# noah-aviel-dove/signals

Measured on AMD Instinct MI355X. Metric: rendered Msamples/s (48 kHz, 256-sample blocks), higher is better.
Workload: dtype f64; 1 GPU; C2: 1024-voice Fixed->Sine->LowPass->Gain->SumBus(stereo) per GPU, 48 kHz, 256-frame blocks, 4096 blocks per batch (f32 storage, f64 phase/recurrence); engine schedule = fused voice chain + bus: sig_fused_voice_bus (Sine->LowPass->Gain->SumBus in ONE launch, its voice tiles added in fixed order by the same kernel; no per-voice sample touches HBM); voices_per_gpu=1024, block_frames=256, start_position=0, parallelism=voices sharded 1024/GPU x1; single process, no collective, rccl_ranks=0

## Files before the change

signals_amd/csrc/fused_voice.hip:

```cpp
#include <cstdlib>

#include "sig_fused_launch.h"

sig_fused::Tuning& sig_fused::tuning() {
    static Tuning t = [] {
        auto env = [](const char* name, int dflt) { const char* e = getenv(name); return e ? atoi(e) : dflt; };
        Tuning u;
        u.vpt = env("SIG_FUSED_VPT", 0); u.span = env("SIG_FUSED_SPAN", 0);
        u.steady = env("SIG_FUSED_STEADY", -1); u.scan = env("SIG_FUSED_SCAN", -1);
        if (u.steady == 2) { u.steady = 1; u.tile_sum_kernel = 1; }
        if (u.steady == 3) { u.steady = 1; u.mix_f32 = 1; }
        return u;
    }();
    return t;
}

namespace {

enum Sink { SINK_VOICES, SINK_MIX, SINK_BUS };
struct FusedCall {
    int osc_kind, filt_type; int32_t rate; int64_t position;
    int32_t block_frames, nblocks, context, voices;
    const double* hertz; int32_t hertz_stride; const double* phase; int32_t phase_stride;
    const double* cutoff; int32_t cutoff_stride; const double* gain; int32_t gain_stride;
    float* out; int64_t out_ld; int32_t* status; void* stream;
    Sink sink = SINK_VOICES;
    bool rows = false;
    int32_t cutoff_rows = 1, gain_rows = 1;
    int pair_op = 0, kind2 = 0;
    const double* hertz2 = nullptr; int32_t hertz2_stride = 0; const double* phase2 = nullptr; int32_t phase2_stride = 0;
    const double* mix = nullptr; int32_t mix_stride = 0;
    int32_t hertz_rows = 1, phase_rows = 1; const double* hertz_hist = nullptr; const double* phase_hist = nullptr;
    bool devpos = false; const int64_t* position_dev = nullptr;
    const float* matrix = nullptr;
    const double* bus_gains = nullptr; int64_t bus_gains_ld = 0; int32_t bus_channels = 0; double* workspace = nullptr;
    double* consts = nullptr; int32_t consts_ready = 0; int force_walk = 0;
};

bool stride_ok(int32_t s) { return (s | 1) == 1; }

bool call_ok(const FusedCall& c)
{
    const bool bus = c.sink == SINK_BUS;
    if (c.filt_type != SIG_FILT_LOWPASS && c.filt_type != SIG_FILT_HIGHPASS) return false;
    if (!(c.rate > 0 && (c.devpos ? c.position_dev != nullptr : c.position >= 0))) return false;
    if (!(c.block_frames >= 0 && c.nblocks >= 0 && c.context >= 0 && c.voices >= 0)) return false;
    if (!(c.hertz && c.cutoff && c.out && c.out_ld >= (bus ? c.bus_channels : c.voices))) return false;
    if (!(stride_ok(c.hertz_stride) && stride_ok(c.phase_stride) && stride_ok(c.cutoff_stride) && stride_ok(c.gain_stride))) return false;
    if (!((c.cutoff_rows == 1 || c.cutoff_rows == c.nblocks) && (c.gain_rows == 1 || c.gain_rows == c.nblocks))) return false;
    if (c.pair_op != 0 && !((c.pair_op == 1 || c.pair_op == 2) && c.kind2 >= SIG_OSC_SINE && c.kind2 <= SIG_OSC_TRIANGLE && c.hertz2 &&
                            stride_ok(c.hertz2_stride) && stride_ok(c.phase2_stride) && stride_ok(c.mix_stride) && (c.pair_op == 2 || c.mix)))
        return false;
    if ((c.hertz_hist || c.phase_hist) && c.block_frames < c.context) return false;
    if (!((c.hertz_rows == 1 || (c.hertz_rows == c.nblocks && c.hertz_hist)) &&
          (c.phase_rows == 1 || (c.phase_rows == c.nblocks && c.phase_hist)) && (!c.phase_hist || c.phase))) return false;
    if (c.sink == SINK_MIX && !(c.matrix && c.voices % 64 == 0)) return false;
    if (bus && !(c.workspace && (c.bus_gains ? c.bus_gains_ld >= c.voices : c.bus_channels == 1))) return false;
    return true;
}

int run_call(const FusedCall& c)
{
    SIG_CHECK_ARG(call_ok(c));
    if (c.block_frames == 0 || c.nblocks == 0 || c.voices == 0) return 0;
    const bool bus = c.sink == SINK_BUS;
    FusedArgs a{c.filt_type, (double)c.rate, c.devpos ? 0 : c.position, c.block_frames, c.nblocks, c.context, c.voices,
                c.hertz, c.hertz_stride, c.phase, c.phase_stride, c.cutoff, c.cutoff_stride, c.gain, c.gain_stride,
                bus ? nullptr : c.out, bus ? 0 : c.out_ld, 0, c.status, c.devpos ? c.position_dev : nullptr};
    a.mix = c.matrix;
    a.consts_ext = c.consts; a.consts_ready = c.consts_ready; a.force_walk = c.force_walk;
    a.cutoff_rows = c.cutoff_rows; a.gain_rows = c.gain_rows;
    a.hertz_rows = c.hertz_rows; a.phase_rows = c.phase_rows; a.hertz_hist = c.hertz_hist; a.phase_hist = c.phase_hist;
    a.pair_op = c.pair_op; a.kind2 = c.kind2; a.hertz2 = c.hertz2; a.hs2 = c.hertz2_stride; a.phase2 = c.phase2; a.ps2 = c.phase2_stride;
    a.mixrow = c.mix; a.ms = c.mix_stride;
    const BusArgs busargs = bus ? BusArgs{c.bus_gains, c.bus_gains_ld, c.workspace, (int64_t)c.block_frames * c.nblocks}
                                : BusArgs{nullptr, 0, nullptr, 0};
    hipStream_t s = static_cast<hipStream_t>(c.stream);
    if (c.rows) {
        SIG_CHECK_ARG(!bus || c.bus_channels == 1 || c.bus_channels == 2);
        return dispatch_rows(bus ? c.bus_channels : 0, c.osc_kind, a, busargs, c.out, c.out_ld, s);
    }
    switch (c.sink) {
        case SINK_BUS: return dispatch_bus(c.gain != nullptr, c.osc_kind, c.bus_channels, a, busargs, c.out, c.out_ld, s);
        case SINK_MIX: return dispatch_mix(c.gain != nullptr, c.osc_kind, a, s);
        default: return dispatch_chain(c.gain != nullptr, c.osc_kind, a, s);
    }
}

void set_rows(FusedCall& c, int32_t cutoff_rows, int32_t gain_rows) { c.rows = true; c.cutoff_rows = cutoff_rows; c.gain_rows = gain_rows; }

void set_bus(FusedCall& c, const double* bus_gains, int64_t bus_gains_ld, int32_t bus_channels, double* workspace)
{
    c.sink = SINK_BUS; c.bus_gains = bus_gains; c.bus_gains_ld = bus_gains_ld; c.bus_channels = bus_channels; c.workspace = workspace;
}
// ... 107 lines not shown
                                      int32_t block_frames, int32_t nblocks, int32_t context, int32_t voices,
                                      const double* hertz, int32_t hertz_stride, int32_t hertz_rows, const double* hertz_hist,
                                      const double* phase, int32_t phase_stride, int32_t phase_rows, const double* phase_hist,
                                      const double* cutoff, int32_t cutoff_stride, int32_t cutoff_rows,
                                      const double* gain, int32_t gain_stride, int32_t gain_rows,
                                      const double* bus_gains, int64_t bus_gains_ld, int32_t bus_channels,
                                      double* workspace, float* out, int64_t out_ld, int32_t* status, void* stream)
{
    FusedCall c{osc_kind, filt_type, rate, position, block_frames, nblocks, context, voices, hertz, hertz_stride, phase, phase_stride,
                cutoff, cutoff_stride, gain, gain_stride, out, out_ld, status, stream};
    set_rows(c, cutoff_rows, gain_rows);
    set_fm(c, hertz_rows, hertz_hist, phase_rows, phase_hist);
    set_bus(c, bus_gains, bus_gains_ld, bus_channels, workspace);
    return run_call(c);
}

extern "C" int sig_fused_osc_biquad_devpos(int osc_kind, int filt_type, int32_t rate, const int64_t* position_dev,
                                           int32_t block_frames, int32_t nblocks, int32_t context, int32_t voices,
                                           const double* hertz, int32_t hertz_stride, const double* phase, int32_t phase_stride,
                                           const double* cutoff, int32_t cutoff_stride,
                                           const double* gain, int32_t gain_stride,
                                           float* out, int64_t out_ld, int32_t* status, void* stream)
{
    FusedCall c{osc_kind, filt_type, rate, 0, block_frames, nblocks, context, voices, hertz, hertz_stride, phase, phase_stride,
                cutoff, cutoff_stride, gain, gain_stride, out, out_ld, status, stream};
    c.devpos = true; c.position_dev = position_dev;
    return run_call(c);
}

namespace {
__global__ void advance_kernel(int64_t* p, int64_t delta) { *p += delta; }
}

extern "C" int sig_advance_position(int64_t* position_dev, int64_t delta, void* stream)
{
    SIG_CHECK_ARG(position_dev != nullptr);
    advance_kernel<<<1, 1, 0, static_cast<hipStream_t>(stream)>>>(position_dev, delta);
    return sig_launch_status();
}

extern "C" int sig_fused_osc_biquad_mix(int osc_kind, int filt_type, int32_t rate, int64_t position,
                                        int32_t block_frames, int32_t nblocks, int32_t context, int32_t voices,
                                        const double* hertz, int32_t hertz_stride, const double* phase, int32_t phase_stride,
                                        const double* cutoff, int32_t cutoff_stride,
                                        const double* gain, int32_t gain_stride,
                                        const float* matrix, float* out, int64_t out_ld, int32_t* status, void* stream)
{
    FusedCall c{osc_kind, filt_type, rate, position, block_frames, nblocks, context, voices, hertz, hertz_stride, phase, phase_stride,
                cutoff, cutoff_stride, gain, gain_stride, out, out_ld, status, stream};
    c.sink = SINK_MIX; c.matrix = matrix;
    return run_call(c);
}

extern "C" int sig_fused_geometry(int32_t voices, int32_t block_frames, int32_t nblocks, int32_t context,
                                  int32_t* voices_per_lane, int32_t* blocks_per_lane)
{
    SIG_CHECK_ARG(voices >= 0 && block_frames >= 0 && nblocks >= 0 && context >= 0 && voices_per_lane && blocks_per_lane);
    FusedArgs a{};
    a.N = block_frames; a.K = nblocks; a.ctx = context; a.voices = voices;
    int vpt = 1, span = 1;
    pick_geometry(a, 4, vpt, span);
    *voices_per_lane = vpt;
    *blocks_per_lane = span;
    return 0;
}

extern "C" int sig_fused_voice_bus_plan(int osc_kind, int64_t position, int32_t voices, int32_t block_frames, int32_t nblocks,
                                       int32_t context, int32_t* voices_per_lane, int32_t* blocks_per_lane,
                                       int32_t* closed_form)
{
    SIG_CHECK_ARG(voices >= 0 && block_frames >= 0 && nblocks >= 0 && context >= 0 && position >= 0);
    SIG_CHECK_ARG(voices_per_lane && blocks_per_lane && closed_form);
    FusedArgs a{};
    a.position = position; a.N = block_frames; a.K = nblocks; a.ctx = context; a.voices = voices;
    const BusPlan p = plan_voice_bus(a, osc_kind);
    *voices_per_lane = p.vpt;
    *blocks_per_lane = p.span;
    *closed_form = p.steady;
    return 0;
}

extern "C" int sig_fused_set_tuning(int32_t voices_per_lane, int32_t blocks_per_lane, int32_t closed_form, int32_t scan)
{
    SIG_CHECK_ARG(voices_per_lane >= 0 && blocks_per_lane >= 0 && closed_form >= -1 && closed_form <= 3 && scan >= -1);
    Tuning& t = tuning();
    t.vpt = voices_per_lane; t.span = blocks_per_lane; t.scan = scan;
    t.steady = (closed_form == 2 || closed_form == 3) ? 1 : closed_form;
    t.tile_sum_kernel = (closed_form == 2) ? 1 : 0;
    t.mix_f32 = (closed_form == 3) ? 1 : 0;
    return 0;
}

extern "C" int64_t sig_fused_voice_bus_workspace(int32_t voices, int64_t rows, int32_t bus_channels)
{
    return (steady_consts_offset(voices, rows, bus_channels) + (int64_t)kSteadyConsts * voices) * (int64_t)sizeof(double);
}

extern "C" int sig_fused_voice_bus(int osc_kind, int filt_type, int32_t rate, int64_t position,
                                   int32_t block_frames, int32_t nblocks, int32_t context, int32_t voices,
                                   const double* hertz, int32_t hertz_stride, const double* phase, int32_t phase_stride,
                                   const double* cutoff, int32_t cutoff_stride,
                                   const double* gain, int32_t gain_stride,
                                   const double* bus_gains, int64_t bus_gains_ld, int32_t bus_channels,
                                   double* workspace, float* out, int64_t out_ld, int32_t* status, void* stream)
{
    FusedCall c{osc_kind, filt_type, rate, position, block_frames, nblocks, context, voices, hertz, hertz_stride, phase, phase_stride,
                cutoff, cutoff_stride, gain, gain_stride, out, out_ld, status, stream};
    set_bus(c, bus_gains, bus_gains_ld, bus_channels, workspace);
    return run_call(c);
}

extern "C" int sig_fused_voice_bus_walk(int osc_kind, int filt_type, int32_t rate, int64_t position,
                                        int32_t block_frames, int32_t nblocks, int32_t context, int32_t voices,
                                        const double* hertz, int32_t hertz_stride, const double* phase, int32_t phase_stride,
                                        const double* cutoff, int32_t cutoff_stride,
                                        const double* gain, int32_t gain_stride,
                                        const double* bus_gains, int64_t bus_gains_ld, int32_t bus_channels,
                                        double* workspace, float* out, int64_t out_ld, int32_t* status, void* stream)
{
    FusedCall c{osc_kind, filt_type, rate, position, block_frames, nblocks, context, voices, hertz, hertz_stride, phase, phase_stride,
                cutoff, cutoff_stride, gain, gain_stride, out, out_ld, status, stream};
    set_bus(c, bus_gains, bus_gains_ld, bus_channels, workspace);
    c.force_walk = 1;
    return run_call(c);
}

extern "C" int64_t sig_fused_voice_consts_size(int32_t voices)
{
    return (int64_t)kSteadyConsts * voices * (int64_t)sizeof(double);
}

extern "C" int sig_fused_voice_bus_prepared(int osc_kind, int filt_type, int32_t rate, int64_t position,
                                            int32_t block_frames, int32_t nblocks, int32_t context, int32_t voices,
                                            const double* hertz, int32_t hertz_stride, const double* phase, int32_t phase_stride,
                                            const double* cutoff, int32_t cutoff_stride,
                                            const double* gain, int32_t gain_stride,
                                            const double* bus_gains, int64_t bus_gains_ld, int32_t bus_channels,
                                            double* workspace, float* out, int64_t out_ld, int32_t* status, void* stream,
                                            double* consts, int32_t consts_ready)
{
    SIG_CHECK_ARG(consts != nullptr);
    FusedCall c{osc_kind, filt_type, rate, position, block_frames, nblocks, context, voices, hertz, hertz_stride, phase, phase_stride,
                cutoff, cutoff_stride, gain, gain_stride, out, out_ld, status, stream};
    set_bus(c, bus_gains, bus_gains_ld, bus_channels, workspace);
    c.consts = consts; c.consts_ready = consts_ready;
    return run_call(c);
}

extern "C" int sig_fused_voice_bus_bound(const sig_fused_voice_bus_call* b, int64_t position, float* out, int32_t consts_ready,
                                         int32_t walk, void* stream)
{
    SIG_CHECK_ARG(b != nullptr && (walk || b->consts != nullptr));
    FusedCall c{b->osc_kind, b->filt_type, b->rate, position, b->block_frames, b->nblocks, b->context, b->voices, b->hertz, b->hertz_stride,
                b->phase, b->phase_stride, b->cutoff, b->cutoff_stride, b->gain, b->gain_stride, out, b->out_ld, b->status, stream};
    set_bus(c, b->bus_gains, b->bus_gains_ld, b->bus_channels, b->workspace);
    if (walk) c.force_walk = 1;
    else { c.consts = b->consts; c.consts_ready = consts_ready; }
    return run_call(c);
}
```

signals_amd/csrc/sig_fused_steady.h:

```cpp
#pragma once
#include <type_traits>

#include "sig_biquad.h"
#include "sig_bus_tile.h"
#include "sig_osc.h"
#include "sig_steady.h"

namespace {

using namespace sig_fused;
using sig_bus::kPairs;
using sig_bus::kTileStride;

enum { SC_NA1, SC_NA2, SC_SCALE, SC_K2C, SC_ST, SC_CT, SC_HRE, SC_HIM, SC_ND, SC_T, SC_T0 = SC_T + 4, kSteadyConsts = SC_T0 + 4 };

__device__ __forceinline__ bool steady_wave(const FusedArgs& a, int v0, int vpt, int64_t p0, int nb) {
    const double q_first = (double)p0 / a.rate, q_last = (double)(p0 + (int64_t)nb * a.N - 1) / a.rate;
    bool ok = true;
    for (int i = 0; i < vpt; ++i) {
        const int v = (v0 + i < a.voices) ? v0 + i : ((v0 < a.voices) ? v0 : 0);
        ok &= steady_voice_ok(a.hertz[(int64_t)v * a.hs], a.phase ? a.phase[(int64_t)v * a.ps] : 0.0, a.rate,
                              a.steady_consts[(int64_t)SC_ST * a.voices + v], q_first, q_last);
    }
    return __all(ok);
}

template <bool GAIN>
__global__ __launch_bounds__(256) void steady_prep_kernel(FusedArgs a, double* __restrict__ consts)
{
    const int v = blockIdx.x * blockDim.x + threadIdx.x;
    if (v >= a.voices) return;
    const SteadyVoice c = steady_constants<GAIN>(a, v);
    if (!c.ok && a.status) atomicOr(a.status, SIG_STATUS_BAD_CUTOFF);
    auto put = [&](int k, double x) { consts[(int64_t)k * a.voices + v] = x; };
    put(SC_NA1, c.na1); put(SC_NA2, c.na2); put(SC_SCALE, c.scale);
    put(SC_K2C, c.k2c); put(SC_ST, c.st); put(SC_CT, c.ct);
    put(SC_HRE, c.hre); put(SC_HIM, c.him); put(SC_ND, c.nd);
    put(SC_T + 0, c.T.a); put(SC_T + 1, c.T.b); put(SC_T + 2, c.T.c); put(SC_T + 3, c.T.d);
    put(SC_T0 + 0, c.T0.a); put(SC_T0 + 1, c.T0.b); put(SC_T0 + 2, c.T0.c); put(SC_T0 + 3, c.T0.d);
}

template <int VPT, int C>
__device__ __forceinline__ void steady_fallback_span(const FusedArgs& a, const BusArgs& bus, double* tile, int lane, int vt,
                                                  int64_t b_first, int nb, int v0)
{
    const int vc = (v0 < a.voices) ? v0 : 0;
    const double* sc = a.steady_consts;
    const double s2 = (a.type == SIG_FILT_LOWPASS) ? 2.0 : -2.0;
    sig_bus::PipelinedTile<C> stage(tile, lane, bus.partials + (int64_t)vt * bus.rows * C, b_first * a.N);
    for (int i = 0; i < VPT; ++i)
        if (v0 + i < a.voices && a.status && sc[(int64_t)SC_NA1 * a.voices + v0 + i] != sc[(int64_t)SC_NA1 * a.voices + v0 + i])
            atomicOr(a.status, SIG_STATUS_BAD_CUTOFF);
#pragma unroll 1
    for (int bi = 0; bi < nb; ++bi) {
        const int64_t p_b = a.position + (b_first + bi) * a.N;
        const int c = (int)((p_b < (int64_t)a.ctx) ? p_b : (int64_t)a.ctx);
        double z0[VPT], z1[VPT];
#pragma unroll
        for (int i = 0; i < VPT; ++i) z0[i] = z1[i] = 0.0;
#pragma unroll 1
        for (int r = -c; r < a.N; ++r) {
            const double q = (double)(p_b + r) / a.rate;
            double acc[C];
#pragma unroll
            for (int ch = 0; ch < C; ++ch) acc[ch] = 0.0;
#pragma unroll
            for (int i = 0; i < VPT; ++i) {
                const bool live = v0 + i < a.voices;
                const int v = live ? v0 + i : vc;
                const double t = q * a.hertz[(int64_t)v * a.hs] + (a.phase ? a.phase[(int64_t)v * a.ps] : 0.0);
                const double x = (double)sig_osc::osc_sine_f32(t);
                double na1 = sc[(int64_t)SC_NA1 * a.voices + v], na2 = sc[(int64_t)SC_NA2 * a.voices + v];
                double scale = live ? sc[(int64_t)SC_SCALE * a.voices + v] : 0.0;
                if (a.cutoff_rows > 1) {
                    Biquad qd;
                    design_butter2(a.type, a.cutoff[(b_first + bi) * (int64_t)(a.cs ? a.voices : 1) + (int64_t)v * a.cs], a.rate, qd);
                    na1 = -qd.a1; na2 = -qd.a2;
                    scale = live ? qd.b0 : 0.0;
                    if (a.gain && a.gain_rows == 1) scale *= a.gain[(int64_t)v * a.gs];
                }
                const double y = x + z0[i];
                z0[i] = fma(na1, y, fma(s2, x, z1[i]));
                z1[i] = fma(na2, y, x);
                if (a.gain_rows > 1) scale *= a.gain[(b_first + bi) * (int64_t)(a.gs ? a.voices : 1) + (int64_t)v * a.gs];
#pragma unroll
                for (int ch = 0; ch < C; ++ch) acc[ch] = fma(bus.pan ? bus.pan[ch * bus.pan_ld + v] * scale : scale, y, acc[ch]);
            }
            if (r >= 0) {
#pragma unroll
                for (int ch = 0; ch < C; ++ch) stage.slot[ch * kTileStride] = acc[ch];
                stage.advance();
            }
        }
    }
    if (stage.staged) stage.now();
}

template <int VPT> struct SteadyVariants {
    static constexpr int count = (VPT >= 8) ? 7 : (VPT == 4) ? 4 : (VPT == 2) ? 3 : 2;
    static constexpr int at(int k) {
        constexpr int v8[7] = {8, 6, 4, 3, 2, 1, 0}, v4[4] = {4, 2, 1, 0}, v2[3] = {2, 1, 0}, v1[2] = {1, 0};
        return (VPT >= 8) ? v8[k] : (VPT == 4) ? v4[k] : (VPT == 2) ? v2[k] : v1[k];
    }
};

#ifndef SIG_STEADY_OCC8
#define SIG_STEADY_OCC8 1
#endif
#ifndef SIG_STEADY_AUTO16
#define SIG_STEADY_AUTO16 0
#endif
#ifndef SIG_STEADY_OCC16
#define SIG_STEADY_OCC16 1
#endif
template <int VPT> struct SteadyOcc { static constexpr int waves = (VPT == 16) ? SIG_STEADY_OCC16 : (VPT == 8) ? SIG_STEADY_OCC8 : 2; };

template <int VPT, int C, bool GROWS, bool CROWS = false>
__device__ __forceinline__ void steady_bus_wave(const FusedArgs& a, const BusArgs& bus, double* tile, int lane, int wave, double* osc_store = nullptr)
{
    constexpr bool OSC_LDS = CROWS && VPT >= 8;
    constexpr int R = kPairs / C;
    constexpr int LC = SteadyVariants<VPT>::at(0);
    static_assert(R % 2 == 0, "the two-term recurrence rotates two registers per voice: row groups are even");
    const int64_t item = (int64_t)blockIdx.x * 4 + wave;
    const int vt = (int)(item % a.voice_tiles);
    const int64_t b_first = (item / a.voice_tiles) * a.span;
    if (b_first >= a.K) return;
    const int nb = (int)((a.K - b_first < (int64_t)a.span) ? a.K - b_first : (int64_t)a.span);
    const int v0 = (vt * SIG_WAVE + lane) * VPT;
    const int vc = (v0 < a.voices) ? v0 : 0;
    const int64_t p0 = a.position + b_first * a.N;
    if (!steady_wave(a, v0, VPT, p0, nb)) {
        steady_fallback_span<VPT, C>(a, bus, tile, lane, vt, b_first, nb, v0);
        return;
    }
    const double* sc = a.steady_consts;

    double na1[LC], na2[LC], k2c[VPT], ya[VPT], yb[VPT], wt[C][VPT];
    int nd_total[VPT];
    const double q_first = (double)p0 / a.rate;
#pragma unroll
    for (int i = 0; i < VPT; ++i) {
        const bool live = v0 + i < a.voices;
        const int v = live ? v0 + i : vc;
        auto cst = [&](int k) { return sc[(int64_t)k * a.voices + v]; };
        const double na1_i = cst(SC_NA1);
        if (i < LC) { na1[i < LC ? i : 0] = na1_i; na2[i < LC ? i : 0] = cst(SC_NA2); }
        k2c[i] = cst(SC_K2C);
        if (live && na1_i != na1_i && a.status) atomicOr(a.status, SIG_STATUS_BAD_CUTOFF);
        const double scale = cst(SC_SCALE);
#pragma unroll
        for (int ch = 0; ch < C; ++ch)
            wt[ch][i] = live ? (bus.pan ? bus.pan[ch * bus.pan_ld + v] * scale : scale) : 0.0;
        const double hz = a.hertz[(int64_t)v * a.hs], ph = a.phase ? a.phase[(int64_t)v * a.ps] : 0.0;
        const double t_first = q_first * hz + ph;
        const double f0 = t_first - rint(t_first);
        const double ur = sin2pi(f0 + 0.25), ui = sin2pi(f0);
        const double hre = cst(SC_HRE), him = cst(SC_HIM);
        const double wr = fma(hre, ur, -(him * ui)), wi = fma(hre, ui, him * ur);
        yb[i] = wi;
        ya[i] = fma(wi, cst(SC_CT), -(wr * cst(SC_ST)));
        const double nd = cst(SC_ND);
        nd_total[i] = (live && nd < (double)kNeverDrops) ? (int)nd : (live ? kNeverDrops : 0);
    }
#pragma unroll
    for (int d = 1; d < SIG_WAVE; d <<= 1) {
        int other[VPT];
#pragma unroll
        for (int i = 0; i < VPT; ++i) other[i] = __shfl_xor(nd_total[i], d, SIG_WAVE);
#pragma unroll
        for (int i = 0; i < VPT; ++i) nd_total[i] = (other[i] > nd_total[i]) ? other[i] : nd_total[i];
    }
#pragma unroll
    for (int i = 0; i < VPT; ++i) nd_total[i] = __builtin_amdgcn_readfirstlane(nd_total[i]);

    double* dstp = bus.partials + (int64_t)vt * bus.rows * C;
    sig_bus::PipelinedTile<C> stage(tile, lane, dstp, b_first * a.N);

    if constexpr (LC < VPT) {
        const int c_min = (b_first == 0 && a.position < (int64_t)a.ctx) ? (int)a.position : a.ctx;
        bool capped = true;
#pragma unroll
        for (int i = LC; i < VPT; ++i) capped &= nd_total[i] <= c_min;
        if (!capped) {
            steady_fallback_span<VPT, C>(a, bus, tile, lane, vt, b_first, nb, v0);
            return;
        }
    }
    [[maybe_unused]] OscPart osc[(CROWS && !OSC_LDS) ? VPT : 1];
    auto osc_slot = [&](int field, int i) -> double& { return osc_store[((size_t)field * VPT + i) * SIG_WAVE + lane]; };
    if constexpr (CROWS) {
#pragma unroll
        for (int i = 0; i < VPT; ++i) {
            const int v = (v0 + i < a.voices) ? v0 + i : vc;
            const OscPart made = steady_osc_part(a.type, a.hertz[(int64_t)v * a.hs], a.rate, a.ctx);
            if constexpr (OSC_LDS) {
                osc_slot(0, i) = made.ct; osc_slot(1, i) = made.st; osc_slot(2, i) = made.beta; osc_slot(3, i) = made.enr; osc_slot(4, i) = made.eni;
            } else {
                osc[i] = made;
            }
        }
    }
    double z0h[LC], z1h[LC];
    auto row = [&](double* sums, int sums_stride, auto m_tag, auto odd_tag) {
        constexpr int M = decltype(m_tag)::value;
        constexpr bool ODD = decltype(odd_tag)::value;
        double y[VPT];
#pragma unroll
        for (int i = 0; i < VPT; ++i) {
            const double ys = ODD ? ya[i] : yb[i];
            if (ODD) yb[i] = fma(k2c[i], ya[i], -yb[i]);
            else ya[i] = fma(k2c[i], yb[i], -ya[i]);
            if (i < M) {
                const int j = i < LC ? i : 0;
                y[i] = ys + z0h[j];
                const double yh = z0h[j];
                z0h[j] = fma(na1[j], yh, z1h[j]);
                z1h[j] = na2[j] * yh;
            } else {
                y[i] = ys;
            }
        }
#pragma unroll
        for (int ch = 0; ch < C; ++ch) {
            double acc = 0.0;
#pragma unroll
            for (int i = 0; i < VPT; ++i) acc = fma(wt[ch][i], y[i], acc);
            sums[ch * sums_stride] = acc;
        }
    };
    sig_bus::FoldedGroup<C> folded(tile, lane, dstp);
    double pend[4];
    int64_t pend_row = 0;
    bool have = false;
    auto rows2 = [&](double* sums, auto m_tag) {
        constexpr int M = decltype(m_tag)::value;
        double y0[VPT], y1[VPT];
#pragma unroll
        for (int i = 0; i < VPT; ++i) {
            y0[i] = yb[i];
            ya[i] = fma(k2c[i], yb[i], -ya[i]);
            y1[i] = ya[i];
            yb[i] = fma(k2c[i], ya[i], -yb[i]);
            if (i < M) {
                const int j = i < LC ? i : 0;
                const double h0 = z0h[j];
                y0[i] += h0;
                const double h1 = fma(na1[j], h0, z1h[j]);
                y1[i] += h1;
                z0h[j] = fma(na1[j], h1, na2[j] * h0);
                z1h[j] = na2[j] * h1;
            }
        }
        double acc0[C], acc1[C];
#pragma unroll
        for (int ch = 0; ch < C; ++ch) { acc0[ch] = 0.0; acc1[ch] = 0.0; }
#pragma unroll
        for (int i = 0; i < VPT; ++i) {
#pragma unroll
            for (int ch = 0; ch < C; ++ch) {
                acc0[ch] = fma(wt[ch][i], y0[i], acc0[ch]);
                acc1[ch] = fma(wt[ch][i], y1[i], acc1[ch]);
            }
        }
#pragma unroll
        for (int ch = 0; ch < C; ++ch) { sums[ch] = acc0[ch]; sums[C + ch] = acc1[ch]; }
    };
    auto group = [&](auto m_tag) {
        double acc[kPairs];
#pragma unroll
        for (int k = 0; k < R; k += 2) {
            rows2(acc + k * C, m_tag);
#pragma unroll
            for (int q = 0; q < kPairs / 4; ++q)
                if (4 * q + 3 < (k + 2) * C && 4 * q + 3 >= k * C)
                    folded.fold4(q, acc[4 * q], acc[4 * q + 1], acc[4 * q + 2], acc[4 * q + 3]);
            if (k + 2 == R / 2 && have) folded.finish(pend, pend_row, R);
        }
        folded.issue(pend);
        pend_row = stage.first; stage.first += R; have = true;
    };
    using Variants = SteadyVariants<VPT>;

    for (int bi = 0; bi < nb; ++bi) {
        if constexpr (GROWS && !CROWS) {
#pragma unroll
            for (int i = 0; i < VPT; ++i) {
                const bool live = v0 + i < a.voices;
                const int v = live ? v0 + i : vc;
                const double scale = sc[(int64_t)SC_SCALE * a.voices + v] * a.gain[(b_first + bi) * (int64_t)(a.gs ? a.voices : 1) + (int64_t)v * a.gs];
#pragma unroll
                for (int ch = 0; ch < C; ++ch) wt[ch][i] = live ? (bus.pan ? bus.pan[ch * bus.pan_ld + v] * scale : scale) : 0.0;
            }
        }
        const bool first = (b_first + bi == 0);
        const int tk = first ? SC_T0 : SC_T;
        const int c = first ? (int)((a.position < (int64_t)a.ctx) ? a.position : (int64_t)a.ctx) : a.ctx;
        if constexpr (CROWS) {
            const int64_t blk = b_first + bi;
            const double q_b = (double)(p0 + (int64_t)bi * a.N) / a.rate;
            double cut_i[VPT], gain_i[VPT];
#pragma unroll
            for (int i = 0; i < VPT; ++i) {
                const int v = (v0 + i < a.voices) ? v0 + i : vc;
                cut_i[i] = a.cutoff[(a.cutoff_rows > 1 ? blk * (int64_t)(a.cs ? a.voices : 1) : 0) + (int64_t)v * a.cs];
                gain_i[i] = a.gain ? a.gain[(a.gain_rows > 1 ? blk * (int64_t)(a.gs ? a.voices : 1) : 0) + (int64_t)v * a.gs] : 1.0;
            }
#pragma unroll
            for (int i = 0; i < VPT; ++i) {
                const bool live = v0 + i < a.voices;
                const int v = live ? v0 + i : vc;
                const double cutoff = cut_i[i], gain = gain_i[i];
                const double hz_v = a.hertz[(int64_t)v * a.hs], ph_v = a.phase ? a.phase[(int64_t)v * a.ps] : 0.0;
                OscPart op;
                if constexpr (OSC_LDS) op = OscPart{osc_slot(0, i), osc_slot(1, i), osc_slot(2, i), osc_slot(3, i), osc_slot(4, i)};
                else op = osc[i];
                if (__builtin_expect(c != a.ctx, 0)) op = steady_osc_part(a.type, hz_v, a.rate, c);
                const double ct_i = op.ct, st_i = op.st;
                const BlockVoice cv = steady_block_constants(a.type, a.rate, cutoff, gain, op, c);
                if (i < LC) { na1[i < LC ? i : 0] = cv.na1; na2[i < LC ? i : 0] = cv.na2; }
                if (live && !cv.ok && a.status) atomicOr(a.status, SIG_STATUS_BAD_CUTOFF);
#pragma unroll
                for (int ch = 0; ch < C; ++ch) wt[ch][i] = live ? (bus.pan ? bus.pan[ch * bus.pan_ld + v] * cv.scale : cv.scale) : 0.0;
                const double t_first = q_b * hz_v + ph_v;
                const double f0 = t_first - rint(t_first);
                const double ur = sin2pi(f0 + 0.25), ui = sin2pi(f0);
                const double wr = fma(cv.hre, ur, -(cv.him * ui)), wi = fma(cv.hre, ui, cv.him * ur);
                yb[i] = wi;
                ya[i] = fma(wi, ct_i, -(wr * st_i));
                if (i < LC) {
                    const double dss = fma(k2c[i], yb[i], -ya[i]) - yb[i];
                    z0h[i < LC ? i : 0] = fma(cv.T.a, yb[i], cv.T.b * dss);
                    z1h[i < LC ? i : 0] = fma(cv.T.c, yb[i], cv.T.d * dss);
                }
                nd_total[i] = (live && cv.nd < (double)kNeverDrops) ? (int)cv.nd : (live ? kNeverDrops : 0);
            }
#pragma unroll
            for (int d = 1; d < SIG_WAVE; d <<= 1) {
                int other[VPT];
#pragma unroll
                for (int i = 0; i < VPT; ++i) other[i] = __shfl_xor(nd_total[i], d, SIG_WAVE);
#pragma unroll
                for (int i = 0; i < VPT; ++i) nd_total[i] = (other[i] > nd_total[i]) ? other[i] : nd_total[i];
            }
#pragma unroll
            for (int i = 0; i < VPT; ++i) nd_total[i] = __builtin_amdgcn_readfirstlane(nd_total[i]);
        }
        int drop_at[LC];
#pragma unroll
        for (int i = 0; i < LC; ++i) {
            drop_at[i] = (nd_total[i] > c) ? nd_total[i] - c : 0;
            if (drop_at[i] > 0) {
                const int v = (v0 + i < a.voices) ? v0 + i : vc;
                const double dss = fma(k2c[i], yb[i], -ya[i]) - yb[i];
                if constexpr (!CROWS) {
                    const double* t = sc + (int64_t)tk * a.voices + v;
                    z0h[i] = fma(t[0], yb[i], t[a.voices] * dss);
                    z1h[i] = fma(t[2 * (int64_t)a.voices], yb[i], t[3 * (int64_t)a.voices] * dss);
                }
            } else {
                z0h[i] = 0.0; z1h[i] = 0.0;
            }
        }
        int done = 0;
        auto single = [&]() {
            row(stage.slot, kTileStride, std::integral_constant<int, LC>{}, std::false_type{});
#pragma unroll
            for (int i = 0; i < VPT; ++i) { const double t = ya[i]; ya[i] = yb[i]; yb[i] = t; }
            ++done;
            stage.advance();
        };
        while (stage.staged != 0 && done < a.N) single();
        const int last_group_row = done + ((a.N - done) / R) * R;
        auto phase = [&](auto k_tag) {
            constexpr int K = decltype(k_tag)::value;
            constexpr int M = Variants::at(K);
            constexpr int lower = (K + 1 < Variants::count) ? Variants::at(K + 1) : 0;
            int until = 0;
#pragma unroll
            for (int i = lower; i < LC; ++i) until = (i < M && drop_at[i] > until) ? drop_at[i] : until;
            if (M == 0) until = a.N;
            until = (until < last_group_row) ? until : last_group_row;
            while (done < until) {
                group(std::integral_constant<int, M>{});
                done += R;
            }
        };
#define SIG_PHASE(K) if constexpr (K < Variants::count) phase(std::integral_constant<int, K>{});
        SIG_PHASE(0) SIG_PHASE(1) SIG_PHASE(2) SIG_PHASE(3) SIG_PHASE(4) SIG_PHASE(5) SIG_PHASE(6) SIG_PHASE(7) SIG_PHASE(8)
#undef SIG_PHASE
        if (done < a.N) {
            if (have) { folded.finish(pend, pend_row, R); have = false; }
#pragma unroll
            for (int i = 0; i < LC; ++i)
                if (drop_at[i] <= done) { z0h[i] = 0.0; z1h[i] = 0.0; }
            while (done < a.N) single();
        }
    }
    if (have) folded.finish(pend, pend_row, R);
    if (stage.staged) stage.now();
}

template <int VPT, int C, bool GROWS = false, bool CROWS = false>
__global__ __launch_bounds__(256) __attribute__((amdgpu_waves_per_eu(CROWS ? 1 : SteadyOcc<VPT>::waves, 8)))
void fused_steady_bus_kernel(FusedArgs a, BusArgs bus)
{
    __shared__ double lds[4][kPairs * kTileStride];
    constexpr bool kOscInLds = CROWS && VPT >= 8;
    __shared__ double osc_lds[kOscInLds ? 4 * 5 * VPT * SIG_WAVE : 1];
    const int lane = threadIdx.x & 63;
    const int wave = __builtin_amdgcn_readfirstlane(threadIdx.x >> 6);
    steady_bus_wave<VPT, C, GROWS, CROWS>(a, bus, lds[wave], lane, wave,
                                          kOscInLds ? osc_lds + (size_t)wave * 5 * VPT * SIG_WAVE : nullptr);
    if (bus.out) sig_bus::sum_tiles_in_workgroup<C>(bus.partials, a.voice_tiles, bus.rows, a.span, a.K, a.N, bus.out, bus.out_ld, lane, wave);
}

int64_t steady_consts_offset(int voices, int64_t rows, int bus_channels) {
    return (int64_t)sig_voice_tiles(voices, 1) * rows * bus_channels;
}

template <bool GAIN, int C, bool GROWS, bool CROWS = false>
int launch_steady(FusedArgs& a, BusArgs& bus, int vpt, float* out, int64_t out_ld, hipStream_t stream)
{
    double* consts = a.consts_ext ? a.consts_ext : bus.partials + steady_consts_offset(a.voices, bus.rows, C);
    a.steady_consts = consts;
    if (!(a.consts_ext && a.consts_ready))
        steady_prep_kernel<GAIN><<<(a.voices + 255) / 256, 256, 0, stream>>>(a, consts);

    a.voice_tiles = sig_voice_tiles(a.voices, vpt);
    unsigned nwg;
    if (!sig_workgroups(sig_span_waves(a.voice_tiles, a.K, a.span), nwg)) return (int)hipErrorInvalidValue;
    if (sig_bus::tiles_sum_in_workgroup(a.voice_tiles) && tuning().tile_sum_kernel == 0) { bus.out = out; bus.out_ld = out_ld; }
    switch (vpt) {
        case 1: fused_steady_bus_kernel<1, C, GROWS, CROWS><<<nwg, 256, 0, stream>>>(a, bus); break;
        case 2: fused_steady_bus_kernel<2, C, GROWS, CROWS><<<nwg, 256, 0, stream>>>(a, bus); break;
        case 8: fused_steady_bus_kernel<8, C, GROWS, CROWS><<<nwg, 256, 0, stream>>>(a, bus); break;
        case 16: if constexpr (!CROWS) { fused_steady_bus_kernel<16, C, GROWS><<<nwg, 256, 0, stream>>>(a, bus); break; }
        default: fused_steady_bus_kernel<4, C, GROWS, CROWS><<<nwg, 256, 0, stream>>>(a, bus); break;
    }
    return sig_launch_status();
}

}
```

signals_amd/csrc/sig_steady.h:

```cpp
#pragma once
#include "sig_biquad.h"
#include "sig_osc.h"

namespace sig_fused {

using sig_biquad::Biquad;
using sig_biquad::design_butter2;

struct FusedArgs {
    int type; double rate; int64_t position; int N, K, ctx, voices;
    const double* hertz; int hs; const double* phase; int ps;
    const double* cutoff; int cs; const double* gain; int gs;
    float* out; int64_t out_ld; int voice_tiles; int* status;
    const int64_t* pos_dev = nullptr;
    const float* mix = nullptr;
    int span = 1;
    int steady = 0;
    const double* steady_consts = nullptr;
    double* consts_ext = nullptr;
    int consts_ready = 0;
    int force_walk = 0;
    int cutoff_rows = 1, gain_rows = 1;
    int hertz_rows = 1, phase_rows = 1;
    const double* hertz_hist = nullptr; const double* phase_hist = nullptr;
    int pair_op = 0, kind2 = 0;
    const double* hertz2 = nullptr; int hs2 = 0; const double* phase2 = nullptr; int ps2 = 0; const double* mixrow = nullptr; int ms = 0;
};

struct BusArgs {
    const double* pan; int64_t pan_ld; double* partials; int64_t rows;
    float* out = nullptr; int64_t out_ld = 0;
};

struct Tuning { int vpt = 0, span = 0, steady = -1, scan = -1, tile_sum_kernel = 0, mix_f32 = 0; };
Tuning& tuning();
int part_b_rows(int C, int kind, const FusedArgs& a, const BusArgs& bus, float* out, int64_t out_ld, hipStream_t s);
int part_b_bus(int gain, int kind, int C, const FusedArgs& a, const BusArgs& bus, float* out, int64_t out_ld, hipStream_t s);
int part_b_mix(int gain, int kind, const FusedArgs& a, hipStream_t s);
int part_b_chain(int gain, int kind, const FusedArgs& a, hipStream_t s);

__device__ __forceinline__ double sin2pi(double f) {
    const double u = fma(f, 2.0, sig_osc::kRoundMagic);
    const double k = u - sig_osc::kRoundMagic;
    const double rq = fma(k, -0.5, f);
    const double y = sig_osc::sin_poly(fma(rq, sig_osc::kTwoPiHi, rq * sig_osc::kTwoPiLo));
    return __hiloint2double(__double2hiint(y) ^ (int)(((unsigned)__double2loint(u) & 1u) << 31), __double2loint(y));
}

struct M2 { double a, b, c, d; };
__device__ __forceinline__ M2 m2_mul(const M2& x, const M2& y) {
    return {fma(x.a, y.a, x.b * y.c), fma(x.a, y.b, x.b * y.d), fma(x.c, y.a, x.d * y.c), fma(x.c, y.b, x.d * y.d)};
}

constexpr double kHomogeneousTol = 1e-9;

__device__ __forceinline__ bool steady_voice_ok(double hz, double ph, double rate, double st, double q_first, double q_last) {
    const double t_first = q_first * hz + ph, t_last = q_last * hz + ph;
    const double d = hz / rate;
    const double dr = d - rint(d);
    return fabs(t_first) < sig_osc::kSineFastMaxT && fabs(t_last) < sig_osc::kSineFastMaxT && fabs(dr) <= 0.25 &&
           fabs(st) >= 1e-3;
}

struct SteadyVoice { bool ok; double na1, na2, scale, k2c, st, ct, hre, him, nd; M2 T, T0; };

template <bool GAIN>
__device__ __forceinline__ SteadyVoice steady_constants_of(const FusedArgs& a, int v, double cutoff, double gain, int c_first)
{
    using sig_biquad::Cx; using sig_biquad::cx_mul; using sig_biquad::cx_div;
    SteadyVoice r;
    Biquad q;
    r.ok = design_butter2(a.type, cutoff, a.rate, q);
    const double s2 = (a.type == SIG_FILT_LOWPASS) ? 2.0 : -2.0;
    const double a1 = q.a1, a2 = q.a2;
    const double d = a.hertz[(int64_t)v * a.hs] / a.rate;
    const double dr = d - rint(d);
    const double st = sin2pi(dr), ct = sin2pi(dr + 0.25), sh = sin2pi(0.5 * dr);
    const Cx z = {ct, -st};
    const Cx z2 = cx_mul(z, z);
    const Cx H = cx_div({1.0 + s2 * z.re + z2.re, s2 * z.im + z2.im}, {1.0 + a1 * z.re + a2 * z2.re, a1 * z.im + a2 * z2.im});
    const Cx P = {H.re - 1.0, H.im};
    const Cx Pe = cx_mul(P, {ct, st});
    const Cx Q = {Pe.re - s2 + a1 * H.re, Pe.im + a1 * H.im};
    const double alpha = 2.0 * sh * sh / st, beta = 1.0 / st;
    auto make_T = [&](int c) {
        const double cf = (double)c * dr;
        const Cx E = cx_div({sin2pi(cf + 0.25), -sin2pi(cf)}, H);
        const Cx PE = cx_mul(P, E), QE = cx_mul(Q, E);
        const M2 Mss = {fma(PE.im, alpha, PE.re), PE.im * beta, fma(QE.im, alpha, QE.re), QE.im * beta};
        M2 Ac = {1.0, 0.0, 0.0, 1.0}, Ap = {-a1, 1.0, -a2, 0.0};
        for (int e = c; e > 0; e >>= 1) {
            if (e & 1) Ac = m2_mul(Ac, Ap);
            Ap = m2_mul(Ap, Ap);
        }
        const M2 t = m2_mul(Ac, Mss);
        return M2{-t.a, -t.b, -t.c, -t.d};
    };
    r.T = make_T(a.ctx);
    r.T0 = (c_first == a.ctx) ? r.T : make_T(c_first);
    r.nd = __builtin_inf();
    {
        const double d2 = a2 - 0.25 * a1 * a1;
        if (r.ok && d2 > 0.0 && a2 > 0.0 && a2 < 1.0) {
            const double dd = sqrt(d2), f2 = 1.0 + 0.25 * a1 * a1 + d2;
            const double kappa = (f2 + sqrt(fmax(f2 * f2 - 4.0 * d2, 0.0))) / (2.0 * dd);
            const double amp = q.b0 * kappa * sqrt(P.re * P.re + P.im * P.im + Q.re * Q.re + Q.im * Q.im);
            const double rows = (amp > kHomogeneousTol) ? log(kHomogeneousTol / amp) / (0.5 * log(a2)) : 0.0;
            if (rows == rows) r.nd = ceil(rows) + 1.0;
        }
    }
    r.na1 = -a1; r.na2 = -a2;
    r.scale = GAIN ? q.b0 * gain : q.b0;
    r.k2c = 2.0 * ct; r.st = st; r.ct = ct; r.hre = H.re; r.him = H.im;
    return r;
}

template <bool GAIN>
__device__ __forceinline__ SteadyVoice steady_constants(const FusedArgs& a, int v)
{
    const int c0 = (int)((a.position < (int64_t)a.ctx) ? a.position : (int64_t)a.ctx);
    return steady_constants_of<GAIN>(a, v, a.cutoff[(int64_t)v * a.cs], GAIN ? a.gain[(int64_t)v * a.gs] : 1.0, c0);
}

struct OscPart { double ct, st, beta, enr, eni; };
struct BlockVoice { bool ok; double na1, na2, scale, hre, him; M2 T; double nd; };

__device__ __forceinline__ OscPart steady_osc_part(int type, double hertz, double rate, int c)
{
    using sig_biquad::Cx; using sig_biquad::cx_mul; using sig_biquad::cx_div;
    const double d = hertz / rate, dr = d - rint(d);
    OscPart o;
    o.st = sin2pi(dr); o.ct = sin2pi(dr + 0.25);
    o.beta = 1.0 / o.st;
    const double s2 = (type == SIG_FILT_LOWPASS) ? 2.0 : -2.0;
    const Cx z = {o.ct, -o.st}, z2 = cx_mul(z, z);
    const Cx N = {1.0 + s2 * z.re + z2.re, s2 * z.im + z2.im};
    const double cf = (double)c * dr;
    const Cx E = cx_div({sin2pi(cf + 0.25), -sin2pi(cf)}, N);
    o.enr = E.re; o.eni = E.im;
    return o;
}

__device__ __forceinline__ BlockVoice steady_block_constants(int type, double rate, double cutoff, double gain, const OscPart& o, int c)
{
    using sig_biquad::Cx; using sig_biquad::cx_mul;
    BlockVoice r;
    double wn = cutoff / (rate * 0.5);
    wn = (wn < 0.0) ? 0.0 : ((wn > 1.0) ? 1.0 : wn);
    r.ok = (wn > 0.0 && wn < 1.0);
    const double x = sig_biquad::kPi * wn * 0.5;
    const double xc = (1.5707963267948966 - x) + 6.123233995736766e-17;
    const double sn = sig_osc::sin_poly(x), cs = sig_osc::sin_poly(xc);
    const double sn2 = sn * sn, cs2 = cs * cs, sc2 = sig_biquad::kSqrt2 * sn * cs;
    const double iden = 1.0 / (cs2 + sc2 + sn2);
    const double b0 = (type == SIG_FILT_LOWPASS) ? sn2 * iden : cs2 * iden;
    double a1 = 2.0 * (sn2 - cs2) * iden, a2 = (cs2 - sc2 + sn2) * iden;
    if (!r.ok) { a1 = a2 = __builtin_nan(""); }
    const double s2 = (type == SIG_FILT_LOWPASS) ? 2.0 : -2.0;
    const Cx z = {o.ct, -o.st};
    const Cx z2 = {o.ct * o.ct - o.st * o.st, -2.0 * o.ct * o.st};
    const Cx N = {1.0 + s2 * z.re + z2.re, s2 * z.im + z2.im}, D = {1.0 + a1 * z.re + a2 * z2.re, a1 * z.im + a2 * z2.im};
    const double id = 1.0 / (D.re * D.re + D.im * D.im);
    const Cx H = {(N.re * D.re + N.im * D.im) * id, (N.im * D.re - N.re * D.im) * id};
    const Cx P = {H.re - 1.0, H.im};
    const Cx Pe = cx_mul(P, {o.ct, o.st});
    const Cx Q = {Pe.re - s2 + a1 * H.re, Pe.im + a1 * H.im};
    const Cx E = cx_mul({o.enr, o.eni}, D);
    const Cx PE = cx_mul(P, E), QE = cx_mul(Q, E);
    const double alpha = (1.0 - o.ct) * o.beta;
    const M2 Mss = {fma(PE.im, alpha, PE.re), PE.im * o.beta, fma(QE.im, alpha, QE.re), QE.im * o.beta};
    M2 Ac;
    const M2 A1 = {-a1, 1.0, -a2, 0.0};
    if (c == 100) {
        const double tr = -a1, det = a2;
        double pw = 1.0, qw = 0.0;
        auto sq = [&]() { const double t = fma(pw, tr, qw + qw), pp = pw * pw; qw = fma(qw, qw, -(pp * det)); pw = pw * t; };
        auto ma = [&]() { const double t = fma(pw, tr, qw); qw = -(pw * det); pw = t; };
        sq(); ma();
        sq(); sq(); sq(); ma();
        sq(); sq();
        Ac = M2{fma(pw, -a1, qw), pw, -a2 * pw, qw};
    } else {
        Ac = M2{1.0, 0.0, 0.0, 1.0};
        M2 Ap = A1;
        for (int e = c; e > 0; e >>= 1) {
            if (e & 1) Ac = m2_mul(Ac, Ap);
            Ap = m2_mul(Ap, Ap);
        }
    }
    const M2 t = m2_mul(Ac, Mss);
    r.T = M2{-t.a, -t.b, -t.c, -t.d};
    r.nd = __builtin_inf();
    {
        const double d2 = a2 - 0.25 * a1 * a1;
        if (r.ok && d2 > 0.0 && a2 > 0.0 && a2 < 1.0) {
            const float dd = __builtin_sqrtf((float)d2);
// ... 27 lines not shown
```

Before: 2.576 million Msamples/s.

## Step steady-state sine recurrence by D rows with precomputed multi-row weights

Adds a stepped variant of the steady closed-form bus kernel that advances each voice's sinusoid recurrence by D (default 4) rows at a time using a cos(D·w) coefficient. Intermediate rows are reconstructed from per-channel history sums, so the per-voice, per-row work becomes a few FMAs into accumulators. Extra per-voice constants (multi-step coefficients, adjusted transient matrices) are precomputed in the prep kernel. Waves whose voices have a small sin(D·w) fall back to the original path, which adds a per-wave check and more registers and risks numerical drift.

```diff
diff --git a/signals_amd/csrc/fused_voice.hip b/signals_amd/csrc/fused_voice.hip
--- a/signals_amd/csrc/fused_voice.hip
+++ b/signals_amd/csrc/fused_voice.hip
@@ -10,6 +10,7 @@
         u.steady = env("SIG_FUSED_STEADY", -1); u.scan = env("SIG_FUSED_SCAN", -1);
         if (u.steady == 2) { u.steady = 1; u.tile_sum_kernel = 1; }
         if (u.steady == 3) { u.steady = 1; u.mix_f32 = 1; }
+        if (u.steady == 4) { u.steady = 1; u.every_row = 1; }
         return u;
     }();
     return t;
@@ -283,10 +284,11 @@
 
 extern "C" int sig_fused_set_tuning(int32_t voices_per_lane, int32_t blocks_per_lane, int32_t closed_form, int32_t scan)
 {
-    SIG_CHECK_ARG(voices_per_lane >= 0 && blocks_per_lane >= 0 && closed_form >= -1 && closed_form <= 3 && scan >= -1);
+    SIG_CHECK_ARG(voices_per_lane >= 0 && blocks_per_lane >= 0 && closed_form >= -1 && closed_form <= 4 && scan >= -1);
     Tuning& t = tuning();
     t.vpt = voices_per_lane; t.span = blocks_per_lane; t.scan = scan;
-    t.steady = (closed_form == 2 || closed_form == 3) ? 1 : closed_form;
+    t.steady = (closed_form >= 2) ? 1 : closed_form;
+    t.every_row = (closed_form == 4) ? 1 : 0;
     t.tile_sum_kernel = (closed_form == 2) ? 1 : 0;
     t.mix_f32 = (closed_form == 3) ? 1 : 0;
     return 0;
diff --git a/signals_amd/csrc/sig_fused_steady.h b/signals_amd/csrc/sig_fused_steady.h
--- a/signals_amd/csrc/sig_fused_steady.h
+++ b/signals_amd/csrc/sig_fused_steady.h
@@ -12,7 +12,11 @@
 using sig_bus::kPairs;
 using sig_bus::kTileStride;
 
-enum { SC_NA1, SC_NA2, SC_SCALE, SC_K2C, SC_ST, SC_CT, SC_HRE, SC_HIM, SC_ND, SC_T, SC_T0 = SC_T + 4, kSteadyConsts = SC_T0 + 4 };
+enum { SC_NA1, SC_NA2, SC_SCALE, SC_K2C, SC_ST, SC_CT, SC_HRE, SC_HIM, SC_ND, SC_T, SC_T0 = SC_T + 4,
+       SC_KJ = SC_T0 + 4,
+       SC_SD = SC_KJ + (kSteadyStep > 1 ? kSteadyStep - 1 : 1),
+       SC_TD, SC_TD0 = SC_TD + 4,
+       kSteadyConsts = SC_TD0 + 4 };
 
 __device__ __forceinline__ bool steady_wave(const FusedArgs& a, int v0, int vpt, int64_t p0, int nb) {
     const double q_first = (double)p0 / a.rate, q_last = (double)(p0 + (int64_t)nb * a.N - 1) / a.rate;
@@ -38,6 +42,25 @@
     put(SC_HRE, c.hre); put(SC_HIM, c.him); put(SC_ND, c.nd);
     put(SC_T + 0, c.T.a); put(SC_T + 1, c.T.b); put(SC_T + 2, c.T.c); put(SC_T + 3, c.T.d);
     put(SC_T0 + 0, c.T0.a); put(SC_T0 + 1, c.T0.b); put(SC_T0 + 2, c.T0.c); put(SC_T0 + 3, c.T0.d);
+    const SteadyStep s = steady_step_constants(a, v, c);
+    for (int j = 2; j <= kSteadyStep; ++j) put(SC_KJ + j - 2, s.kj[j - 2]);
+    put(SC_SD, s.sd);
+    put(SC_TD + 0, s.TD.a); put(SC_TD + 1, s.TD.b); put(SC_TD + 2, s.TD.c); put(SC_TD + 3, s.TD.d);
+    put(SC_TD0 + 0, s.TD0.a); put(SC_TD0 + 1, s.TD0.b); put(SC_TD0 + 2, s.TD0.c); put(SC_TD0 + 3, s.TD0.d);
+}
+
+template <int VPT>
+__device__ __forceinline__ bool steady_step_wave(const FusedArgs& a, int lane, int wave) {
+    const int64_t item = (int64_t)blockIdx.x * 4 + wave;
+    const int vt = (int)(item % a.voice_tiles);
+    const int v0 = (vt * SIG_WAVE + lane) * VPT;
+    bool ok = true;
+#pragma unroll
+    for (int i = 0; i < VPT; ++i) {
+        const int v = (v0 + i < a.voices) ? v0 + i : ((v0 < a.voices) ? v0 : 0);
+        ok &= a.steady_consts[(int64_t)SC_SD * a.voices + v] >= kSteadyStepMinSin;
+    }
+    return __all(ok);
 }
 
 template <int VPT, int C>
@@ -115,13 +138,17 @@
 #endif
 template <int VPT> struct SteadyOcc { static constexpr int waves = (VPT == 16) ? SIG_STEADY_OCC16 : (VPT == 8) ? SIG_STEADY_OCC8 : 2; };
 
-template <int VPT, int C, bool GROWS, bool CROWS = false>
+template <int VPT, int C, bool GROWS, bool CROWS = false, int STEP = 1>
 __device__ __forceinline__ void steady_bus_wave(const FusedArgs& a, const BusArgs& bus, double* tile, int lane, int wave, double* osc_store = nullptr)
 {
     constexpr bool OSC_LDS = CROWS && VPT >= 8;
     constexpr int R = kPairs / C;
     constexpr int LC = SteadyVariants<VPT>::at(0);
     static_assert(R % 2 == 0, "the two-term recurrence rotates two registers per voice: row groups are even");
+    constexpr int D = STEP;
+    static_assert(D == 1 || (!GROWS && !CROWS && LC == VPT && D == kSteadyStep && R % (2 * D) == 0),
+                  "stepped row groups: constant bus weights, and an even number of D-row sub-groups per group (the roles of ya / yb "
+                  "and of the history registers swap per sub-group: a group ends in the layout in which it began)");
     const int64_t item = (int64_t)blockIdx.x * 4 + wave;
     const int vt = (int)(item % a.voice_tiles);
     const int64_t b_first = (item / a.voice_tiles) * a.span;
@@ -137,6 +164,13 @@
     const double* sc = a.steady_consts;
 
     double na1[LC], na2[LC], k2c[VPT], ya[VPT], yb[VPT], wt[C][VPT];
+    [[maybe_unused]] double wj[D > 1 ? D - 1 : 1][C][VPT], hist[D > 1 ? D - 1 : 1][C];
+    if constexpr (D > 1) {
+#pragma unroll
+        for (int j = 0; j < D - 1; ++j)
+#pragma unroll
+            for (int ch = 0; ch < C; ++ch) hist[j][ch] = 0.0;
+    }
     int nd_total[VPT];
     const double q_first = (double)p0 / a.rate;
 #pragma unroll
@@ -146,7 +180,7 @@
         auto cst = [&](int k) { return sc[(int64_t)k * a.voices + v]; };
         const double na1_i = cst(SC_NA1);
         if (i < LC) { na1[i < LC ? i : 0] = na1_i; na2[i < LC ? i : 0] = cst(SC_NA2); }
-        k2c[i] = cst(SC_K2C);
+        k2c[i] = cst(D > 1 ? SC_KJ + D - 2 : SC_K2C);
         if (live && na1_i != na1_i && a.status) atomicOr(a.status, SIG_STATUS_BAD_CUTOFF);
         const double scale = cst(SC_SCALE);
 #pragma unroll
@@ -160,6 +194,22 @@
         const double wr = fma(hre, ur, -(him * ui)), wi = fma(hre, ui, him * ur);
         yb[i] = wi;
         ya[i] = fma(wi, cst(SC_CT), -(wr * cst(SC_ST)));
+        if constexpr (D > 1) {
+            const double k1 = cst(SC_K2C);
+            double nxt = yb[i], cur = ya[i];
+#pragma unroll
+            for (int j = 1; j < D; ++j) {
+                const double cj = (j == 1) ? k1 : cst(SC_KJ + (j > 1 ? j - 2 : 0));
+#pragma unroll
+                for (int ch = 0; ch < C; ++ch) {
+                    wj[j - 1][ch][i] = wt[ch][i] * cj;
+                    hist[j - 1][ch] = fma(wt[ch][i], cur, hist[j - 1][ch]);
+                }
+                const double before = fma(k1, cur, -nxt);
+                nxt = cur; cur = before;
+            }
+            ya[i] = cur;
+        }
         const double nd = cst(SC_ND);
         nd_total[i] = (live && nd < (double)kNeverDrops) ? (int)nd : (live ? kNeverDrops : 0);
     }
@@ -266,8 +316,80 @@
 #pragma unroll
         for (int ch = 0; ch < C; ++ch) { sums[ch] = acc0[ch]; sums[C + ch] = acc1[ch]; }
     };
+    auto rowsD = [&](double* sums, auto m_tag, auto odd_tag) {
+        constexpr int M = decltype(m_tag)::value;
+        constexpr bool ODD = decltype(odd_tag)::value;
+        double yc[VPT], y0[VPT], h[D > 1 ? D - 1 : 1][M > 0 ? M : 1];
+#pragma unroll
+        for (int i = 0; i < VPT; ++i) {
+            if (ODD) { yc[i] = ya[i]; yb[i] = fma(k2c[i], ya[i], -yb[i]); }
+            else { yc[i] = yb[i]; ya[i] = fma(k2c[i], yb[i], -ya[i]); }
+            y0[i] = yc[i];
+            if (i < M) {
+                const int s = i < LC ? i : 0;
+                const int m = i < M ? i : 0;
+                double h0 = z0h[s], h1 = fma(na1[s], h0, z1h[s]);
+                y0[i] += h0;
+                h[0][m] = h1;
+#pragma unroll
+                for (int j = 2; j < D; ++j) {
+                    const double hj = fma(na1[s], h1, na2[s] * h0);
+                    h[j > 1 ? j - 1 : 0][m] = hj;
+                    h0 = h1; h1 = hj;
+                }
+                z0h[s] = fma(na1[s], h1, na2[s] * h0);
+                z1h[s] = na2[s] * h1;
+            }
+        }
+        double acc[D][C];
+#pragma unroll
+        for (int ch = 0; ch < C; ++ch) {
+            acc[0][ch] = 0.0;
+#pragma unroll
+            for (int j = 1; j < D; ++j) acc[j][ch] = -hist[(ODD ? D - j : j) - 1][ch];
+        }
+#pragma unroll
+        for (int i = 0; i < VPT; ++i) {
+#pragma unroll
+            for (int ch = 0; ch < C; ++ch) {
+                acc[0][ch] = fma(wt[ch][i], y0[i], acc[0][ch]);
+#pragma unroll
+                for (int j = 1; j < D; ++j) acc[j][ch] = fma(wj[j - 1][ch][i], yc[i], acc[j][ch]);
+            }
+        }
+#pragma unroll
+        for (int ch = 0; ch < C; ++ch)
+#pragma unroll
+            for (int j = 1; j < D; ++j) hist[(ODD ? D - j : j) - 1][ch] = acc[j][ch];
+#pragma unroll
+        for (int i = 0; i < M; ++i) {
+#pragma unroll
+            for (int ch = 0; ch < C; ++ch)
+#pragma unroll
+                for (int j = 1; j < D; ++j) acc[j][ch] = fma(wt[ch][i], h[j - 1][i], acc[j][ch]);
+        }
+#pragma unroll
+        for (int j = 0; j < D; ++j)
+#pragma unroll
+            for (int ch = 0; ch < C; ++ch) sums[j * C + ch] = acc[j][ch];
+    };
     auto group = [&](auto m_tag) {
         double acc[kPairs];
+        if constexpr (D > 1) {
+#pragma unroll
+            for (int k = 0; k < R; k += D) {
+                if ((k / D) % 2 == 0) rowsD(acc + k * C, m_tag, std::false_type{});
+                else rowsD(acc + k * C, m_tag, std::true_type{});
+#pragma unroll
+                for (int q = 0; q < kPairs / 4; ++q)
+                    if (4 * q + 3 < (k + D) * C && 4 * q + 3 >= k * C)
+                        folded.fold4(q, acc[4 * q], acc[4 * q + 1], acc[4 * q + 2], acc[4 * q + 3]);
+                if (k + D == R / 2 && have) folded.finish(pend, pend_row, R);
+            }
+            folded.issue(pend);
+            pend_row = stage.first; stage.first += R; have = true;
+            return;
+        }
 #pragma unroll
         for (int k = 0; k < R; k += 2) {
             rows2(acc + k * C, m_tag);
@@ -294,7 +416,7 @@
             }
         }
         const bool first = (b_first + bi == 0);
-        const int tk = first ? SC_T0 : SC_T;
+        const int tk = (D > 1) ? (first ? SC_TD0 : SC_TD) : (first ? SC_T0 : SC_T);
         const int c = first ? (int)((a.position < (int64_t)a.ctx) ? a.position : (int64_t)a.ctx) : a.ctx;
         if constexpr (CROWS) {
             const int64_t blk = b_first + bi;
@@ -352,7 +474,7 @@
             drop_at[i] = (nd_total[i] > c) ? nd_total[i] - c : 0;
             if (drop_at[i] > 0) {
                 const int v = (v0 + i < a.voices) ? v0 + i : vc;
-                const double dss = fma(k2c[i], yb[i], -ya[i]) - yb[i];
+                const double dss = (D > 1) ? ya[i] : fma(k2c[i], yb[i], -ya[i]) - yb[i];
                 if constexpr (!CROWS) {
                     const double* t = sc + (int64_t)tk * a.voices + v;
                     z0h[i] = fma(t[0], yb[i], t[a.voices] * dss);
@@ -370,7 +492,7 @@
             ++done;
             stage.advance();
         };
-        while (stage.staged != 0 && done < a.N) single();
+        if constexpr (D == 1) while (stage.staged != 0 && done < a.N) single();
         const int last_group_row = done + ((a.N - done) / R) * R;
         auto phase = [&](auto k_tag) {
             constexpr int K = decltype(k_tag)::value;
@@ -389,7 +511,7 @@
 #define SIG_PHASE(K) if constexpr (K < Variants::count) phase(std::integral_constant<int, K>{});
         SIG_PHASE(0) SIG_PHASE(1) SIG_PHASE(2) SIG_PHASE(3) SIG_PHASE(4) SIG_PHASE(5) SIG_PHASE(6) SIG_PHASE(7) SIG_PHASE(8)
 #undef SIG_PHASE
-        if (done < a.N) {
+        if (D == 1 && done < a.N) {
             if (have) { folded.finish(pend, pend_row, R); have = false; }
 #pragma unroll
             for (int i = 0; i < LC; ++i)
@@ -398,10 +520,12 @@
         }
     }
     if (have) folded.finish(pend, pend_row, R);
-    if (stage.staged) stage.now();
-}
-
-template <int VPT, int C, bool GROWS = false, bool CROWS = false>
+    if (D == 1 && stage.staged) stage.now();
+}
+
+constexpr int steady_step_of(int C) { return ((kPairs / C) % (2 * kSteadyStep) == 0) ? kSteadyStep : 1; }
+
+template <int VPT, int C, bool GROWS = false, bool CROWS = false, int STEP = 1>
 __global__ __launch_bounds__(256) __attribute__((amdgpu_waves_per_eu(CROWS ? 1 : SteadyOcc<VPT>::waves, 8)))
 void fused_steady_bus_kernel(FusedArgs a, BusArgs bus)
 {
@@ -410,6 +534,10 @@
     __shared__ double osc_lds[kOscInLds ? 4 * 5 * VPT * SIG_WAVE : 1];
     const int lane = threadIdx.x & 63;
     const int wave = __builtin_amdgcn_readfirstlane(threadIdx.x >> 6);
+    if constexpr (STEP > 1) {
+        if (a.steady != 4 && steady_step_wave<VPT>(a, lane, wave)) steady_bus_wave<VPT, C, GROWS, CROWS, STEP>(a, bus, lds[wave], lane, wave);
+        else steady_bus_wave<VPT, C, GROWS, CROWS>(a, bus, lds[wave], lane, wave);
+    } else
     steady_bus_wave<VPT, C, GROWS, CROWS>(a, bus, lds[wave], lane, wave,
                                           kOscInLds ? osc_lds + (size_t)wave * 5 * VPT * SIG_WAVE : nullptr);
     if (bus.out) sig_bus::sum_tiles_in_workgroup<C>(bus.partials, a.voice_tiles, bus.rows, a.span, a.K, a.N, bus.out, bus.out_ld, lane, wave);
@@ -431,6 +559,14 @@
     unsigned nwg;
     if (!sig_workgroups(sig_span_waves(a.voice_tiles, a.K, a.span), nwg)) return (int)hipErrorInvalidValue;
     if (sig_bus::tiles_sum_in_workgroup(a.voice_tiles) && tuning().tile_sum_kernel == 0) { bus.out = out; bus.out_ld = out_ld; }
+    constexpr int STEP = (GROWS || CROWS) ? 1 : steady_step_of(C);
+    if constexpr (STEP > 1) {
+        if (vpt == 8 && a.N % (kPairs / C) == 0) {
+            if (tuning().every_row) a.steady = 4;
+            fused_steady_bus_kernel<8, C, false, false, STEP><<<nwg, 256, 0, stream>>>(a, bus);
+            return sig_launch_status();
+        }
+    }
     switch (vpt) {
         case 1: fused_steady_bus_kernel<1, C, GROWS, CROWS><<<nwg, 256, 0, stream>>>(a, bus); break;
         case 2: fused_steady_bus_kernel<2, C, GROWS, CROWS><<<nwg, 256, 0, stream>>>(a, bus); break;
diff --git a/signals_amd/csrc/sig_steady.h b/signals_amd/csrc/sig_steady.h
--- a/signals_amd/csrc/sig_steady.h
+++ b/signals_amd/csrc/sig_steady.h
@@ -32,7 +32,7 @@
     float* out = nullptr; int64_t out_ld = 0;
 };
 
-struct Tuning { int vpt = 0, span = 0, steady = -1, scan = -1, tile_sum_kernel = 0, mix_f32 = 0; };
+struct Tuning { int vpt = 0, span = 0, steady = -1, scan = -1, tile_sum_kernel = 0, mix_f32 = 0, every_row = 0; };
 Tuning& tuning();
 int part_b_rows(int C, int kind, const FusedArgs& a, const BusArgs& bus, float* out, int64_t out_ld, hipStream_t s);
 int part_b_bus(int gain, int kind, int C, const FusedArgs& a, const BusArgs& bus, float* out, int64_t out_ld, hipStream_t s);
@@ -112,6 +112,29 @@
     r.na1 = -a1; r.na2 = -a2;
     r.scale = GAIN ? q.b0 * gain : q.b0;
     r.k2c = 2.0 * ct; r.st = st; r.ct = ct; r.hre = H.re; r.him = H.im;
+    return r;
+}
+
+#ifndef SIG_STEADY_STEP
+#define SIG_STEADY_STEP 4
+#endif
+constexpr int kSteadyStep = SIG_STEADY_STEP;
+static_assert(kSteadyStep == 1 || kSteadyStep == 2 || kSteadyStep == 4, "row groups are written for tone steps of 1, 2 and 4 rows");
+constexpr double kSteadyStepMinSin = 1e-3;
+
+struct SteadyStep { double kj[kSteadyStep > 1 ? kSteadyStep - 1 : 1], sd; M2 TD, TD0; };
+
+__device__ __forceinline__ SteadyStep steady_step_constants(const FusedArgs& a, int v, const SteadyVoice& c)
+{
+    const double d = a.hertz[(int64_t)v * a.hs] / a.rate;
+    const double dr = d - rint(d);
+    SteadyStep r;
+    for (int j = 2; j <= kSteadyStep; ++j) r.kj[j - 2] = 2.0 * sin2pi((double)j * dr + 0.25);
+    const double sD = sin2pi((double)kSteadyStep * dr), cD = sin2pi((double)kSteadyStep * dr + 0.25), sh = sin2pi(0.5 * dr);
+    r.sd = fabs(sD);
+    const double q = c.st / sD, A = fma(q, cD, -2.0 * sh * sh);
+    auto from = [&](const M2& T) { return M2{fma(T.b, A, T.a), -(T.b * q), fma(T.d, A, T.c), -(T.d * q)}; };
+    r.TD = from(c.T); r.TD0 = from(c.T0);
     return r;
 }
 
```

Result: no change. 2.589 million Msamples/s, median of 6 (+0.5%).
